# vertgenlab/gonomics

Measured on AMD Instinct MI355X. Metric: DP cells/sec + aligned pairs/sec, affine-gap 150bp x 10kb batch, higher is better.
Workload: dtype int32

## Files before the change

gonomics_amd/_lib.py:

```python
import ctypes
import os

import numpy as np

_HERE = os.path.dirname(os.path.abspath(__file__))
LIB_PATH = os.environ.get("GNX_LIB_PATH") or os.path.join(_HERE, "libgonomics_align_hip.so")

GNX_OK, GNX_EINVAL, GNX_EBASE, GNX_EEMPTY, GNX_ERANGE, GNX_EDEVICE, GNX_ENOMEM, GNX_ECAPACITY, GNX_ETRACE, GNX_EDIVZERO, GNX_ESTALE = range(11)
GNX_AFFINE_GAP, GNX_CONST_GAP, GNX_AFFINE_GAP_HIGHMEM, GNX_AFFINE_GAP_LOCAL, GNX_CONST_GAP_HIGHMEM = range(5)

EXPORTS = ["gnx_device_count", "gnx_init", "gnx_shutdown", "gnx_last_error", "gnx_free", "gnx_align_batch",
           "gnx_align_batch_windows", "gnx_align_pair", "gnx_align_batch_device", "gnx_get_timing",
           "gnx_affine_gap_chunk_batch", "gnx_multiple_affine_gap_batch", "gnx_gsw_extend_batch",
           "gnx_init_devices", "gnx_n_devices", "gnx_set_reference", "gnx_set_reference_synthetic", "gnx_align_batch_by_offset",
           "gnx_seed_index_build", "gnx_seed_index_set", "gnx_seed_find_batch", "gnx_seed_index_set_gen", "gnx_seed_find_batch_gen", "gnx_gsw_graph_create", "gnx_gsw_graph_free", "gnx_gsw_map_reads", "gnx_debug_occupy", "gnx_debug_counter", "gnx_debug_fill_scratch", "gnx_debug_gapless_certificate", "gnx_debug_gapless_certificate_n", "gnx_reference_info",
           "gnx_score_batch", "gnx_score_batch_windows", "gnx_score_batch_by_offset", "gnx_score_batch_device",
           "gnx_locate_batch", "gnx_locate_batch_windows", "gnx_locate_batch_by_offset",
           "gnx_locate_span_batch", "gnx_locate_span_batch_windows", "gnx_locate_span_batch_by_offset",
           "gnx_affine_gap_chunk_score_batch", "gnx_multiple_affine_gap_score_batch",
           "gnx_best_of_by_offset", "gnx_best_of_windows", "gnx_best_pair_by_offset", "gnx_best_pair_windows",
           "gnx_reference_index_build", "gnx_reference_index_info", "gnx_reference_index_get", "gnx_seed_candidates",
           "gnx_summarize_batch", "gnx_summarize_batch_windows", "gnx_summarize_batch_by_offset",
           "gnx_md_batch", "gnx_md_batch_windows", "gnx_md_batch_by_offset", "gnx_mapq_batch",
           "gnx_pileup_open", "gnx_pileup_info", "gnx_pileup_add_by_offset", "gnx_pileup_get", "gnx_pileup_calls", "gnx_pileup_close",
           "gnx_pileup_track_alleles", "gnx_pileup_allele_info", "gnx_pileup_alleles", "gnx_pileup_indel_calls",
           "gnx_pileup_alleles_norm", "gnx_pileup_indel_calls_norm",
           "gnx_pileup_track_qualities", "gnx_pileup_qual_info", "gnx_pileup_add_by_offset_qual", "gnx_pileup_get_qual", "gnx_pileup_genotypes"]
GNX_XCOL_EQ, GNX_XCOL_X = 3, 4


class GnxCigar(ctypes.Structure):
    _fields_ = [("run_length", ctypes.c_int64), ("op", ctypes.c_uint8), ("_pad", ctypes.c_uint8 * 7)]


CIGAR_DTYPE = np.dtype({"names": ["run_length", "op"], "formats": [np.int64, np.uint8], "offsets": [0, 8], "itemsize": 16})


class GnxParams(ctypes.Structure):
    _fields_ = [("mode", ctypes.c_int32), ("_reserved", ctypes.c_int32), ("scores", ctypes.c_int64 * 25),
                ("gap_open", ctypes.c_int64), ("gap_extend", ctypes.c_int64),
                ("checkersize_i", ctypes.c_int64), ("checkersize_j", ctypes.c_int64)]


class GnxTiming(ctypes.Structure):
    _fields_ = [("fill_ms", ctypes.c_double), ("traceback_ms", ctypes.c_double), ("total_ms", ctypes.c_double),
                ("cells", ctypes.c_int64), ("n_launches", ctypes.c_int64), ("trace_bytes", ctypes.c_int64),
                ("dominant_ms", ctypes.c_double), ("dominant_launches", ctypes.c_int64), ("fast_path", ctypes.c_int32),
                ("_pad", ctypes.c_int32), ("host_ms", ctypes.c_double), ("stage0_ms", ctypes.c_double), ("fetch_ms", ctypes.c_double),
# ... 202 lines not shown
            L.gnx_pileup_genotypes.argtypes = [ctypes.POINTER(GnxGenoOpts), ctypes.POINTER(c_p), ctypes.POINTER(i64)]
            L.gnx_pileup_genotypes.restype = ctypes.c_int
        L.gnx_seed_index_build.argtypes = [c_p, c_p, i64, ctypes.c_int, ctypes.c_int, ctypes.POINTER(c_p), ctypes.POINTER(c_p), ctypes.POINTER(i64)]
        L.gnx_seed_index_build.restype = ctypes.c_int
        L.gnx_seed_index_set.argtypes = [c_p, c_p, i64, c_p, c_p, i64, ctypes.c_int]
        L.gnx_seed_index_set.restype = ctypes.c_int
        L.gnx_seed_find_batch.argtypes = [c_p, c_p, i64, ctypes.POINTER(c_p), ctypes.POINTER(c_p)]
        L.gnx_seed_find_batch.restype = ctypes.c_int
        L.gnx_seed_index_set_gen.argtypes = [c_p, c_p, i64, c_p, c_p, i64, ctypes.c_int, ctypes.POINTER(ctypes.c_uint64)]
        L.gnx_seed_index_set_gen.restype = ctypes.c_int
        L.gnx_seed_find_batch_gen.argtypes = [ctypes.c_uint64, c_p, c_p, i64, ctypes.POINTER(c_p), ctypes.POINTER(c_p)]
        L.gnx_seed_find_batch_gen.restype = ctypes.c_int
        if hasattr(L, "gnx_gsw_map_reads"):
            L.gnx_gsw_graph_create.argtypes = [c_p, c_p, i64, c_p, c_p, i64, ctypes.c_int, ctypes.c_int, ctypes.POINTER(c_p)]
            L.gnx_gsw_graph_create.restype = ctypes.c_int
            L.gnx_gsw_graph_free.argtypes = [c_p]
            L.gnx_gsw_graph_free.restype = None
            L.gnx_gsw_map_reads.argtypes = [c_p, c_p, c_p, i64, ctypes.c_int, c_p, i64, ctypes.c_int, ctypes.POINTER(c_p), ctypes.POINTER(c_p), ctypes.POINTER(c_p)]
            L.gnx_gsw_map_reads.restype = ctypes.c_int
        L.gnx_get_timing.argtypes = [ctypes.POINTER(GnxTiming)]
        L.gnx_get_timing.restype = ctypes.c_int
        if hasattr(L, "gnx_debug_occupy"):
            L.gnx_debug_occupy.argtypes = [ctypes.c_int, ctypes.c_int]
            L.gnx_debug_occupy.restype = ctypes.c_int
        if hasattr(L, "gnx_debug_counter"):
            L.gnx_debug_counter.argtypes = [ctypes.c_int, ctypes.c_int, ctypes.POINTER(ctypes.c_int64)]
            L.gnx_debug_counter.restype = ctypes.c_int
        if hasattr(L, "gnx_debug_gapless_certificate"):
            L.gnx_debug_gapless_certificate.argtypes = [ctypes.POINTER(GnxParams), c_p, i64, c_p, i64, i64, c_p]
            L.gnx_debug_gapless_certificate.restype = ctypes.c_int
        if hasattr(L, "gnx_debug_gapless_certificate_n"):
            L.gnx_debug_gapless_certificate_n.argtypes = [ctypes.POINTER(GnxParams), c_p, i64, c_p, i64, i64, c_p]
            L.gnx_debug_gapless_certificate_n.restype = ctypes.c_int
        if hasattr(L, "gnx_debug_fill_scratch"):
            L.gnx_debug_fill_scratch.argtypes = [ctypes.c_uint32, ctypes.POINTER(ctypes.c_int64), ctypes.POINTER(ctypes.c_int64)]
            L.gnx_debug_fill_scratch.restype = ctypes.c_int
        _lib = L
    return _lib


def debug_counter(which=0, reset=True):
    v = ctypes.c_int64()
    check(lib().gnx_debug_counter(which, 1 if reset else 0, ctypes.byref(v)))
    return int(v.value)


def debug_fill_scratch(pattern):
    nb, by = ctypes.c_int64(), ctypes.c_int64()
    check(lib().gnx_debug_fill_scratch(ctypes.c_uint32(int(pattern) & 0xFFFFFFFF), ctypes.byref(nb), ctypes.byref(by)))
    return int(nb.value), int(by.value)


def debug_gapless_certificate(params, a, b, K=16):
    a = np.ascontiguousarray(a, dtype=np.uint8)
    b = np.ascontiguousarray(b, dtype=np.uint8)
    out = np.zeros(4, dtype=np.int64)
    check(lib().gnx_debug_gapless_certificate(ctypes.byref(params), a.ctypes.data, a.shape[0], b.ctypes.data, b.shape[0], int(K), out.ctypes.data))
    return bool(out[0]), int(out[1]), int(out[2]), int(out[3])


def debug_gapless_certificate_n(params, a, b, K=16):
    a = np.ascontiguousarray(a, dtype=np.uint8)
    b = np.ascontiguousarray(b, dtype=np.uint8)
    out = np.zeros(6, dtype=np.int64)
    check(lib().gnx_debug_gapless_certificate_n(ctypes.byref(params), a.ctypes.data, a.shape[0], b.ctypes.data, b.shape[0], int(K), out.ctypes.data))
    return bool(out[0]), int(out[1]), int(out[2]), int(out[3]), bool(out[4]), int(out[5])


def check(rc):
    if rc != GNX_OK:
        raise GnxError(rc, lib().gnx_last_error().decode("utf-8", "replace"))


def make_params(mode, scores, gap_open, gap_extend=0, checkersize_i=10000, checkersize_j=10000):
    p = GnxParams()
    p.mode = mode
    flat = [int(v) for row in scores for v in row]
    if len(flat) != 25:
        raise ValueError("scores must be a 5x5 matrix")
    for k, v in enumerate(flat):
        p.scores[k] = v
    p.gap_open = int(gap_open)
    p.gap_extend = int(gap_extend)
    p.checkersize_i = int(checkersize_i)
    p.checkersize_j = int(checkersize_j)
    return p


def _u8(a):
    return np.ascontiguousarray(a, dtype=np.uint8)


def _i64(a):
    return np.ascontiguousarray(a, dtype=np.int64)


def _take(ops_p, off_p, n_pairs):
    L = lib()
    off = np.ctypeslib.as_array(ctypes.cast(off_p, ctypes.POINTER(ctypes.c_int64)), shape=(n_pairs + 1,)).copy()
# ... 847 lines not shown
```

gonomics_amd/csrc/fp_cert.hip.h:

```cpp
#pragma once
#include "gnx_common.hip.h"
#include "fp_cert_decide.h"

namespace {
constexpr int CERT_K = 16;
constexpr int CERT_SLOTS = 512;
constexpr int CERT_NMAX = 160;
constexpr int CERT_CHUNK = (CERT_NMAX + 63) / 64;

__device__ __forceinline__ int64_t cert_wave_sum(int64_t v) {
#pragma unroll
    for (int d = 32; d >= 1; d >>= 1) v += __shfl_xor(v, d, 64);
    return v;
}
__device__ __forceinline__ int64_t cert_wave_scan(int64_t v, int lane) {
#pragma unroll
    for (int d = 1; d < 64; d <<= 1) { const int64_t t = __shfl_up(v, d, 64); if (lane >= d) v += t; }
    return v;
}

__device__ __forceinline__ unsigned cert_hash(unsigned code) { return code * 0x9E3779B1u; }
__device__ __forceinline__ unsigned cert_pack4(unsigned w) {
    unsigned x = w & 0x03030303u;
    x = (x | (x >> 6)) & 0x000F000Fu;
    return (x | (x >> 12)) & 0xFFu;
}

template <bool PK>
__global__ __launch_bounds__(64) void fp_cert_kernel(const PairPlan *__restrict__ plans, int n_pairs,
                                                     const uint8_t *__restrict__ a_buf, const int64_t *__restrict__ a_start,
                                                     const uint8_t *__restrict__ b_buf, const int64_t *__restrict__ b_start,
                                                     KParams kp, TbParams tp, GnxCertMatrix mx, gnx_cigar *__restrict__ stage, int cap,
                                                     int64_t *__restrict__ score_out, int64_t *__restrict__ nops,
                                                     int64_t *__restrict__ live, int64_t *__restrict__ n_cert, int *__restrict__ err) {
    __shared__ unsigned keys[CERT_SLOTS];
    __shared__ int qv[CERT_SLOTS];
    __shared__ unsigned filt[CERT_SLOTS];
    __shared__ uint8_t sa[CERT_NMAX];
    __shared__ int64_t sw[40];
    const int p = (int)blockIdx.x;
    if (p >= n_pairs) return;
    const int lane = threadIdx.x;
    const PairPlan pl = plans[p];
    const int n = pl.n, m = pl.m;
    bool bad = false;
    bool out = n < CERT_K || n > CERT_NMAX || m < n + 2 || kp.o4 >= 0 || tp.ci < n || tp.cj < m;
    BetaSrcT<PK ? 1 : 0> bp;
    const int64_t boff = b_start[pl.src];
    bp.init(b_buf, kp, boff, m);
    if (PK && bp.dirty) out = true;
    if (out) { if (lane == 0) live[p] = 1; return; }
// ... 84 lines not shown
    int64_t loss[CERT_CHUNK];
#pragma unroll
    for (int k = 0; k < CERT_CHUNK; k++) {
        const int i = i0 + k;
        loss[k] = 0;
        if (k < chunk && i < n) loss[k] = gnx_certn_lane_row<8>(&ln, sw, mx.R[4], 1, i, sa[i], (unsigned)bp.at(c + i), (unsigned)bp.at(i), (unsigned)bp.at(m - n + i));
    }
    if (__any(!ln.ok)) { if (lane == 0) live[p] = 1; return; }
    int nu = 0;
#pragma unroll
    for (int k = 0; k < CERT_CHUNK; k++) nu += __popcll(__ballot(ln.nn > k));
    const int64_t D = cert_wave_sum(ln.loss), mid_sum = cert_wave_sum(ln.mid);
    const int64_t Fi = cert_wave_scan(ln.f, lane), Gi = cert_wave_scan(ln.g, lane);
    const int f_pos = __any(ln.rows > 0 && Fi - ln.f + ln.f_top > 0);
    int64_t g_low = ln.rows > 0 ? Gi - ln.g + ln.g_low : INT64_MAX;
    int g_row = ln.rows > 0 ? ln.g_row : n;
#pragma unroll
    for (int d = 32; d >= 1; d >>= 1) gnx_cert_low_min(&g_low, &g_row, __shfl_xor(g_low, d, 64), __shfl_xor(g_row, d, 64));
    const GnxCertBounds t = gnx_certn_bounds(mx.lambda, mx.o, n, CERT_K, D, nu);
    int64_t h1 = 0, h2 = 0, t1 = 0, t2 = 0;
    if (t.edge) {
#pragma unroll
        for (int k = 0; k < CERT_CHUNK; k++) {
            const int i = i0 + k;
            if (i < t.T1) h1 += loss[k];
            if (i < t.T2) h2 += loss[k];
            if (i >= n - t.T1) t1 += loss[k];
            if (i >= n - t.T2) t2 += loss[k];
        }
        h1 = cert_wave_sum(h1); h2 = cert_wave_sum(h2); t1 = cert_wave_sum(t1); t2 = cert_wave_sum(t2);
    }
    int64_t best, ds, sc;
    gnx_cert_tail(__shfl(Gi, 63, 64), g_low, g_row, n, &best, &ds);
    if (!gnx_cert_finish(&t, mx.o, mx.e, n, m, f_pos, mid_sum, h1, h2, t1, t2, best, ds, &ds, &sc)) { if (lane == 0) live[p] = 1; return; }
    if (lane == 0) {
        gnx_cigar *stg = stage + (int64_t)p * cap;
        int cnt = 0;
        auto put = [&](int op, int64_t run) { gnx_cigar g; g.run_length = run; g.op = (uint8_t)op; for (int z = 0; z < 7; z++) g._pad[z] = 0; stg[cnt++] = g; };
        if (ds > 0) put(0, ds);
        put(1, (int64_t)m - n - c);
        put(0, (int64_t)n - ds);
        put(1, c);
        nops[p] = cnt;
        score_out[p] = sc;
        live[p] = 0;
        if (nu > 0) atomicAdd(reinterpret_cast<unsigned long long *>(n_cert), 1ull);
    }
}

__global__ __launch_bounds__(256) void fp_cert_gather_kernel(int n_pairs, const int64_t *__restrict__ live, const int64_t *__restrict__ off,
                                                             const PairPlan *__restrict__ plans, int *__restrict__ list, PairPlan *__restrict__ out) {
    const int p = blockIdx.x * blockDim.x + threadIdx.x;
    if (p >= n_pairs || !live[p]) return;
    const int64_t k = off[p];
    list[k] = p;
    out[k] = plans[p];
}

}
```

gonomics_amd/csrc/fp_cert_decide.h:

```cpp
#pragma once
#include <stdint.h>

#if defined(__HIPCC__) || defined(__CUDACC__)
#define GNX_CERT_HD __host__ __device__
#else
#define GNX_CERT_HD
#endif

struct GnxCertMatrix {
    int64_t w[25];
    int64_t R[5];
    int64_t lambda;
    int64_t o, e;
    int32_t ok;
};

GNX_CERT_HD inline void gnx_cert_matrix_init(GnxCertMatrix *mx, const int64_t *scores, int64_t gap_open, int64_t gap_extend) {
    mx->o = gap_open; mx->e = gap_extend;
    for (int x = 0; x < 25; x++) mx->w[x] = scores[x] - 2 * gap_extend;
    int ok = gap_open < 0 ? 1 : 0;
    int64_t lam = INT64_MAX;
    for (int x = 0; x < 4; x++) {
        const int64_t Rx = mx->w[x * 5 + x];
        int64_t worst = INT64_MIN;
        for (int y = 0; y < 5; y++) if (y != x && mx->w[x * 5 + y] > worst) worst = mx->w[x * 5 + y];
        mx->R[x] = Rx;
        if (Rx <= 0 || Rx <= worst) ok = 0;
        const int64_t loss = Rx - worst < Rx ? Rx - worst : Rx;
        if (loss < lam) lam = loss;
    }
    int64_t rn = 0;
    for (int y = 0; y < 5; y++) if (mx->w[20 + y] > rn) rn = mx->w[20 + y];
    mx->R[4] = rn;
    mx->lambda = lam;
    mx->ok = (ok && lam > 0) ? 1 : 0;
}

GNX_CERT_HD inline int64_t gnx_cert_table8_entry(const GnxCertMatrix *mx, int k) { return (k & 7) < 5 ? mx->w[(k >> 3) * 5 + (k & 7)] : 0; }

struct GnxCertRow {
// ... 98 lines not shown
        nu += a[i] == 4 ? 1 : 0;
        deficit += r.loss;
        mid_sum += r.mid;
        F += r.f;
        if (F > 0) return 0;
    }
    const GnxCertBounds t = gnx_certn_bounds(mx->lambda, mx->o, n, K, deficit, nu);
    if (!t.ok) return 0;
    int64_t h1 = 0, h2 = 0, t1 = 0, t2 = 0;
    if (t.edge)
        for (int64_t i = 0; i < t.T2; i++) {
            const int64_t j = n - 1 - i;
            gnx_certn_row<5>(mx->w, rn, allow_n, a[i], bd[i], bf[i], bl[i], &r);
            gnx_certn_row<5>(mx->w, rn, allow_n, a[j], bd[j], bf[j], bl[j], &r2);
            h2 += r.loss; t2 += r2.loss;
            if (i < t.T1) { h1 += r.loss; t1 += r2.loss; }
        }
    int64_t G = 0, best = 0, ds = 0;
    for (int64_t d = 1; d <= n; d++) {
        const int64_t i = n - d;
        gnx_certn_row<5>(mx->w, rn, allow_n, a[i], bd[i], bf[i], bl[i], &r);
        G += r.g;
        if (G >= best) { best = G; ds = d; }
    }
    if (edge) *edge = t.edge;
    if (nu_out) *nu_out = nu;
    return gnx_cert_finish(&t, mx->o, mx->e, n, m, 0, mid_sum, h1, h2, t1, t2, best, ds, d_star, score);
}
GNX_CERT_HD inline int gnx_cert_decide(const GnxCertMatrix *mx, const uint8_t *a, int64_t n, const uint8_t *bd, const uint8_t *bf, const uint8_t *bl,
                                       int64_t m, int64_t c, int64_t K, int64_t ci, int64_t cj, int64_t *d_star, int64_t *score) {
    return gnx_certn_decide(mx, a, n, bd, bf, bl, m, c, K, ci, cj, 0, d_star, score, nullptr, nullptr);
}

inline int gnx_cert_scan_naive(const uint8_t *a, int64_t n, const uint8_t *b, int64_t m, int64_t K, int64_t *c_out) {
    int found = 0;
    int64_t c = 0;
    for (int64_t q = 0; q + K <= n; q++)
        for (int64_t j = 0; j + K <= m; j++) {
            int64_t t = 0;
            while (t < K && a[q + t] < 4 && a[q + t] == (b[j + t] & 3)) t++;
            if (t < K) continue;
            if (found && j - q != c) return 0;
            found = 1; c = j - q;
        }
    *c_out = c;
    return found;
}
```

gonomics_amd/csrc/gnx_align.hip:

```cpp
#include "gnx_common.hip.h"
#include "fill_affine.hip.h"
#include "fp_sweep.hip.h"
#include "fp_rounds.h"
#include "fill_const.hip.h"
#include "traceback.hip.h"
#include "fp_walk.hip.h"
#include "fp_cert.hip.h"
#include "aux_kernels.hip.h"
#include "const_long.hip.h"
#include "const_long_wg.hip.h"
#include "const_long_walk.hip.h"
#include "affine_long.hip.h"
#include "affine_long64.hip.h"
#include "const_long64.hip.h"
#include "farm64.hip.h"
#include "lat_fill.hip.h"
#include "lat_wide.hip.h"
#include "seed_kernels.hip.h"
#include "score_sweep.hip.h"
#include "n1_sweep.hip.h"
#include "span_origin.hip.h"
#include "ref_seeds.hip.h"
#include "aln_summary.hip.h"
#include "aln_md.hip.h"
// ... 172 lines not shown
    for (int x = 0; x < 25; x++) if (p->scores[x] > lim || p->scores[x] < -lim) { set_err("score out of int32 kernel range%s", ""); return GNX_ERANGE; }
    if (p->gap_open > lim || p->gap_open < -lim || (affine && (p->gap_extend > lim || p->gap_extend < -lim))) { set_err("gap penalty out of int32 kernel range%s", ""); return GNX_ERANGE; }
    kp.b2 = nullptr; kp.bflag = nullptr; kp.brank = nullptr; kp.bexc = nullptr;
    for (int x = 0; x < 25; x++) kp.sc4[x] = (int)(4 * p->scores[x]);
    kp.o4 = (int)(4 * p->gap_open);
    kp.e4 = affine ? (int)(4 * p->gap_extend) : 0;
    kp.oe4 = kp.o4 + kp.e4;
    kp.d00_4 = local ? 0 : kp.o4;
    kp.ecol4 = local ? 0 : kp.e4;
    kp.g4 = kp.o4;
    kp.rb_pub = RB_PUB;
    kp.ckc = CKC_SMALL;
    tp.ci = lowmem ? p->checkersize_i : ((int64_t)1 << 62);
    tp.cj = lowmem ? p->checkersize_j : ((int64_t)1 << 62);
    tp.d00 = local ? 0 : p->gap_open;
    tp.ecol = local ? 0 : p->gap_extend;
    tp.gap_open = p->gap_open;
    tp.gap_extend = affine ? p->gap_extend : 0;
    tp.affine = affine ? 1 : 0;
    return GNX_OK;
}

int64_t max_abs_pen(const gnx_params *p, bool affine) {
    int64_t mx = 0;
    for (int x = 0; x < 25; x++) mx = std::max<int64_t>(mx, llabs((long long)p->scores[x]));
    if (affine) mx = std::max<int64_t>(mx, llabs((long long)(p->gap_open + p->gap_extend)));
    mx = std::max<int64_t>(mx, llabs((long long)p->gap_open));
    if (affine) mx = std::max<int64_t>(mx, llabs((long long)p->gap_extend));
    return mx;
}

std::atomic<int64_t> g_cert_ok{0}, g_cert_offered{0};
std::atomic<int64_t> g_cert_n{0};
std::atomic<int64_t> g_fpc_hit{0}, g_fpc_miss{0};

int run_device(const gnx_params *prm, int64_t n_pairs, const uint8_t *d_a, const int64_t *d_as, const uint8_t *d_b, const int64_t *d_bs,
               const int64_t *h_alen, const int64_t *h_blen, int64_t *d_score, gnx_cigar *d_ops, int64_t ops_capacity, int64_t *d_ops_off,
               int64_t *out_total, hipStream_t stream, const int *d_smat, const int64_t *h_soff, int gsw, int2 *d_endpos, bool no_fast_path, bool smat16);

__global__ __launch_bounds__(64) void occupy_kernel(long long ticks) {
    extern __shared__ int occupy_lds[];
    occupy_lds[threadIdx.x] = (int)ticks;
    const long long t0 = wall_clock64();
    while (wall_clock64() - t0 < ticks) __builtin_amdgcn_s_sleep(64);
}

int claim_test_switch(int *sw, hipStream_t st) {
    const char *e = getenv("GNX_TICKET_DELAY"), *g = getenv("GNX_CLAIM_GRACE_US");
    if (!e || !*e) return GNX_OK;
    const int v = (std::min(std::max(atoi(e), 0), 0xffff)) | ((g && *g) ? (std::min(std::max(atoi(g), 1), 0x7fff) << 16) : 0);
    HIPCHK(hipMemcpyAsync(sw, &v, 4, hipMemcpyHostToDevice, st));
    HIPCHK(hipStreamSynchronize(st));
    return GNX_OK;
}

int launch_scan(const int64_t *d_nops, int n, int64_t *d_off, int64_t *d_carry, hipStream_t stream) {
    Ctx &c = g_ctx;
    if (n <= 8192) { hipLaunchKernelGGL(scan_kernel, dim3(1), dim3(1024), 0, stream, d_nops, n, d_off, d_carry); return GNX_OK; }
    const int nb = (n + 1023) / 1024;
    int rc;
    if ((rc = c.scan_tmp.ensure((size_t)(2 * nb + 2) * 8))) return rc;
    int64_t *sums = reinterpret_cast<int64_t *>(c.scan_tmp.p), *boff = sums + nb;
    hipLaunchKernelGGL(scan_sums_kernel, dim3((unsigned)nb), dim3(1024), 0, stream, d_nops, n, sums);
    hipLaunchKernelGGL(scan_kernel, dim3(1), dim3(1024), 0, stream, sums, nb, boff, d_carry);
    hipLaunchKernelGGL(scan_apply_kernel, dim3((unsigned)nb), dim3(1024), 0, stream, d_nops, n, boff, d_off);
    return GNX_OK;
// ... 74 lines not shown
    if (!cached || c.fpc_ptr != c.plans.p) {
        if (cached) { set_err("internal: plan cache lost its buffer%s", ""); return GNX_EINVAL; }
        HIPCHK(hipMemcpyAsync(c.plans.p, plans.data(), (size_t)np * sizeof(PairPlan), hipMemcpyHostToDevice, stream));
        HIPCHK(hipStreamSynchronize(stream));
        c.fpc_alen.assign(h_alen, h_alen + n_pairs); c.fpc_blen.assign(h_blen, h_blen + n_pairs);
        c.fpc_roff = roff; c.fpc_coff = coff; c.fpc_cells = cells; c.fpc_mmax = m_maxb; c.fpc_ptr = c.plans.p; c.fpc_rboff = rboff; c.fpc_strips = S;
    }
    (cached ? g_fpc_hit : g_fpc_miss)++;
    const PairPlan *dpl = reinterpret_cast<const PairPlan *>(c.plans.p);
    int *d_hfwd = reinterpret_cast<int *>(c.hcol.p);
    int *d_whcol = d_hfwd + np;
    unsigned *d_rowi = reinterpret_cast<unsigned *>(c.fp_rowi.p);
    unsigned *d_tail = reinterpret_cast<unsigned *>(c.fp_tail.p);
    int2 *d_ckpt = reinterpret_cast<int2 *>(c.fp_ckpt.p);
    FpState *d_st = reinterpret_cast<FpState *>(c.fp_states.p);
    gnx_cigar *d_stage = reinterpret_cast<gnx_cigar *>(c.fp_stage.p);
    int64_t *d_nops = reinterpret_cast<int64_t *>(c.nops.p);
    PairPlan *d_wpl[2] = {reinterpret_cast<PairPlan *>(c.fp_wplans[0].p), reinterpret_cast<PairPlan *>(c.fp_wplans[1].p)};
    int *d_act[2] = {reinterpret_cast<int *>(c.fp_active[0].p), reinterpret_cast<int *>(c.fp_active[1].p)};
    const dim3 blockF(64), blockT(64);
    const int max_it = getenv("GNX_FP_MAXIT") ? atoi(getenv("GNX_FP_MAXIT")) : -1;
    const int tiles_per = (int)((m_maxb + FP_TILE - 1) / FP_TILE);
    double refill_ms = 0;

    const char *certenv = getenv("GNX_FP_CERT");
    const bool cert = S == 1 && !xp && prm->gap_open < 0 && !(certenv && certenv[0] == '0') &&
                      ((certenv && certenv[0] == '2') || n_pairs > (int64_t)G8 * 3 * 4 * c.n_cu);
    int n_live = np;
    int64_t *d_cflag = nullptr, *d_coff = nullptr;
    int *d_live = nullptr;
    PairPlan *d_gpl = nullptr;
    bool gathered = false;
    if (cert) {
        if ((rc = c.fp_cflag.ensure((size_t)(2 * np + 3) * 8))) return rc;
        if ((rc = c.fp_live.ensure((size_t)np * 4))) return rc;
        if ((rc = c.fp_gplans.ensure((size_t)np * sizeof(PairPlan)))) return rc;
        d_cflag = reinterpret_cast<int64_t *>(c.fp_cflag.p); d_coff = d_cflag + np + 2;
        d_live = reinterpret_cast<int *>(c.fp_live.p);
        d_gpl = reinterpret_cast<PairPlan *>(c.fp_gplans.p);
    }
    auto certify = [&](hipStream_t st) -> int {
        GnxCertMatrix mx;
        int64_t sc64[25];
        for (int x = 0; x < 25; x++) sc64[x] = (int64_t)(kp.sc4[x] >> 2);
        gnx_cert_matrix_init(&mx, sc64, (int64_t)(kp.o4 >> 2), (int64_t)(kp.e4 >> 2));
        g_cert_offered += np;
        if (!mx.ok) return GNX_OK;
        HIPCHK(hipMemsetAsync(d_cflag + np, 0, 16, st));
        auto kc = kp.b2 ? fp_cert_kernel<true> : fp_cert_kernel<false>;
        hipLaunchKernelGGL(kc, dim3((unsigned)np), dim3(64), 0, st, dpl, np, d_a, d_as, d_b, d_bs, kp, tp, mx, d_stage, CAP, d_score, d_nops, d_cflag, d_cflag + np + 1, d_err);
        HIPCHK(hipGetLastError());
        if ((rc = launch_scan(d_cflag, np, d_coff, d_cflag + np, st))) return rc;
        hipLaunchKernelGGL(fp_cert_gather_kernel, dim3((unsigned)((np + 255) / 256)), dim3(256), 0, st, np, d_cflag, d_coff, dpl, d_live, d_gpl);
        HIPCHK(hipGetLastError());
        int64_t nl[2] = {0, 0};
        HIPCHK(hipMemcpyAsync(nl, d_cflag + np, 16, hipMemcpyDeviceToHost, st));
        HIPCHK(hipStreamSynchronize(st));
        n_live = (int)nl[0];
        gathered = true;
        g_cert_ok += np - n_live - nl[1];
        g_cert_n += nl[1];
        if (getenv("GNX_DEBUG")) fprintf(stderr, "[gnx fp] gapless certificate: %d of %d pairs certified (%d of them hold an N), %d go through the sweep\n", np - n_live, np, (int)nl[1], n_live);
        return GNX_OK;
    };

    auto forward = [&](const PairPlan *splans, int cnt, hipStream_t st) -> int {
        if (cnt <= 0) return GNX_OK;
        const dim3 grid8((unsigned)((cnt + G8 - 1) / G8));
        if (two) {
            int2 *rb = reinterpret_cast<int2 *>(c.rowbuf.p);
            const int top_rows = (int)(top_hi + G8 - 1) / G8;
            const bool pk = kp.b2 != nullptr;
            auto klev = xp ? (top_rows <= 8 ? fp_sweep_levels_kernel<8, true> : (top_rows <= 12 ? fp_sweep_levels_kernel<12, true> : (top_rows <= 16 ? fp_sweep_levels_kernel<16, true> : fp_sweep_levels_kernel<20, true>)))
                      : pk ? (top_rows <= 8 ? fp_sweep_levels_kernel<8, false, true> : (top_rows <= 12 ? fp_sweep_levels_kernel<12, false, true> : (top_rows <= 16 ? fp_sweep_levels_kernel<16, false, true> : fp_sweep_levels_kernel<20, false, true>)))
                           : (top_rows <= 8 ? fp_sweep_levels_kernel<8> : (top_rows <= 12 ? fp_sweep_levels_kernel<12> : (top_rows <= 16 ? fp_sweep_levels_kernel<16> : fp_sweep_levels_kernel<20>)));
            const int W = (int)grid8.x;
            int *prog = reinterpret_cast<int *>(c.fp_prog.p);
            if (!no_pipe()) {
                HIPCHK(hipMemsetAsync(prog, 0, ((size_t)S * W * 2 + 2) * 4, st));
                if ((rc = claim_test_switch(prog + (size_t)S * W * 2, st))) return rc;
                hipLaunchKernelGGL(klev, dim3((unsigned)(S * W)), blockF, 0, st, splans, cnt, d_a, d_as, d_b, d_bs, kp, d_hfwd, d_ckpt, d_rowi, d_tail, d_err, rb, S, W, 0, 1, prog);
                HIPCHK(hipGetLastError());
                int e = 0;
                HIPCHK(hipMemcpyAsync(&e, d_err, 4, hipMemcpyDeviceToHost, st));
                HIPCHK(hipStreamSynchronize(st));
                if (!(e & 16)) return GNX_OK;
                e &= ~16;
                HIPCHK(hipMemcpyAsync(d_err, &e, 4, hipMemcpyHostToDevice, st));
                HIPCHK(hipStreamSynchronize(st));
                if (getenv("GNX_DEBUG")) fprintf(stderr, "[gnx fp] a row block timed out waiting for the one above it -> one launch per level\n");
            }
            for (int level = 0; level < S; level++)
                hipLaunchKernelGGL(klev, grid8, blockF, 0, st, splans, cnt, d_a, d_as, d_b, d_bs, kp, d_hfwd, d_ckpt, d_rowi, d_tail, d_err, rb, S, W, level, 0, prog);
            HIPCHK(hipGetLastError());
            return GNX_OK;
// ... 3357 lines not shown
    if (rc) return rc;
    if (!a || !b || !out || n < 1 || m < 1 || K < 1 || !affine || local) { set_err("bad argument%s", ""); return GNX_EINVAL; }
    out[0] = out[1] = out[2] = out[3] = 0;
    GnxCertMatrix mx;
    gnx_cert_matrix_init(&mx, p->scores, p->gap_open, p->gap_extend);
    int64_t c = 0, ds = 0, sc = 0;
    for (int64_t j = 0; j < m; j++) if (b[j] >= 5) return GNX_OK;
    if (m < n + 2 || K > n || !gnx_cert_scan_naive(a, n, b, m, K, &c)) return GNX_OK;
    if (c <= 0 || c >= m - n) return GNX_OK;
    if (!gnx_cert_decide(&mx, a, n, b + c, b, b + (m - n), m, c, K, tp.ci, tp.cj, &ds, &sc)) return GNX_OK;
    out[0] = 1; out[1] = c; out[2] = ds; out[3] = sc;
    return GNX_OK;
}

int gnx_debug_gapless_certificate_n(const gnx_params *p, const uint8_t *a, int64_t n, const uint8_t *b, int64_t m, int64_t K, int64_t *out) {
    g_err[0] = 0;
    if (!getenv("GNX_DEBUG_ENTRY")) { set_err("gnx_debug_gapless_certificate_n is a test hook: set GNX_DEBUG_ENTRY=1%s", ""); return GNX_EINVAL; }
    KParams kp; TbParams tp; bool affine, local, lowmem;
    int rc = check_params(p, kp, tp, affine, local, lowmem);
    if (rc) return rc;
    if (!a || !b || !out || n < 1 || m < 1 || K < 1 || !affine || local) { set_err("bad argument%s", ""); return GNX_EINVAL; }
    for (int x = 0; x < 6; x++) out[x] = 0;
    GnxCertMatrix mx;
    gnx_cert_matrix_init(&mx, p->scores, p->gap_open, p->gap_extend);
    int64_t c = 0, ds = 0, sc = 0, edge = 0, nu = 0;
    for (int64_t j = 0; j < m; j++) if (b[j] >= 5) return GNX_OK;
    if (m < n + 2 || K > n || !gnx_cert_scan_naive(a, n, b, m, K, &c)) return GNX_OK;
    if (c <= 0 || c >= m - n) return GNX_OK;
    if (!gnx_certn_decide(&mx, a, n, b + c, b, b + (m - n), m, c, K, tp.ci, tp.cj, 1, &ds, &sc, &edge, &nu)) return GNX_OK;
    out[0] = 1; out[1] = c; out[2] = ds; out[3] = sc; out[4] = edge; out[5] = nu;
    return GNX_OK;
}

int gnx_debug_counter(int which, int reset, int64_t *out) {
    ApiCall api;
    CtxScope sc(ctx_at(0));
    if (which < 0 || which > 13 || !out) { set_err("bad argument%s", ""); return GNX_EINVAL; }
    if (which >= 12) {
        std::atomic<int64_t> &v = which == 12 ? g_fpc_hit : g_fpc_miss;
        *out = v.load();
        if (reset) v = 0;
        return GNX_OK;
    }
    if (which >= 9) {
        std::atomic<int64_t> &v = which == 9 ? g_cert_ok : (which == 10 ? g_cert_offered : g_cert_n);
        *out = v.load();
        if (reset) v = 0;
        return GNX_OK;
    }
    if (which >= 7) {
        std::atomic<int64_t> &v = which == 7 ? g_sv_lds : g_sv_slab;
        *out = v.load();
        if (reset) v = 0;
        return GNX_OK;
    }
    if (which == 1 || which == 2) {
        *out = which == 1 ? g_pq_batches.load() : g_pq_pairs.load();
        if (reset) { if (which == 1) g_pq_batches = 0; else g_pq_pairs = 0; }
        return GNX_OK;
    }
    if (which >= 5) { *out = which == 5 ? g_last_w64_r.load() : g_last_w64_ck.load(); return GNX_OK; }
    int rc = ensure_init();
    if (rc) return rc;
    HIPCHK(hipSetDevice(g_ctx.device));
    HIPCHK(hipDeviceSynchronize());
    unsigned long long v = 0;
    if (which >= 3) {
        unsigned long long q[2] = {0, 0};
        HIPCHK(hipMemcpyFromSymbol(q, HIP_SYMBOL(g_dev_q1), sizeof(q)));
        if (reset) { const unsigned long long z[2] = {0, 0}; HIPCHK(hipMemcpyToSymbol(HIP_SYMBOL(g_dev_q1), z, sizeof(z))); }
// ... 20 lines not shown
```

include/gnx_align.h:

```cpp
#ifndef GNX_ALIGN_H
#define GNX_ALIGN_H

#include <stdint.h>

#ifdef __cplusplus
extern "C" {
#endif

#define GNX_OK 0
#define GNX_EINVAL 1
#define GNX_EBASE 2
#define GNX_EEMPTY 3
#define GNX_ERANGE 4
#define GNX_EDEVICE 5
#define GNX_ENOMEM 6
#define GNX_ECAPACITY 7
#define GNX_ETRACE 8
#define GNX_EDIVZERO 9
#define GNX_ESTALE 10

#define GNX_COL_M 0
#define GNX_COL_I 1
#define GNX_COL_D 2

// ... 224 lines not shown
    int32_t  depth;
    uint8_t  ref, _pad2[3];
} gnx_pile_indel_call;
int gnx_pileup_track_alleles(int64_t reserve_events);
int gnx_pileup_allele_info(int32_t *out_tracking, int64_t *out_events, int64_t *out_device_bytes);
int gnx_pileup_alleles(gnx_pile_allele **out, int64_t *out_n);
int gnx_pileup_indel_calls(const gnx_pile_call_opts *o, gnx_pile_indel_call **out_calls, int64_t *out_n);
int gnx_pileup_alleles_norm(gnx_pile_allele **out, int64_t *out_n);
int gnx_pileup_indel_calls_norm(const gnx_pile_call_opts *o, gnx_pile_indel_call **out_calls, int64_t *out_n);

typedef struct gnx_geno_opts { int32_t min_depth, min_qual, prior_het, prior_hom, _reserved[2]; } gnx_geno_opts;
typedef struct gnx_pile_genotype {
    int64_t pos;
    int32_t pl[3];
    int32_t gq, qual;
    int32_t depth, ref_count, alt_count, alt_fwd;
    uint8_t gt, ref, alt, _pad;
} gnx_pile_genotype;
int gnx_pileup_track_qualities(int32_t min_baseq);
int gnx_pileup_qual_info(int32_t *out_tracking, int32_t *out_min_baseq, int64_t *out_device_bytes);
int gnx_pileup_add_by_offset_qual(const gnx_params *p, int64_t n_pairs, const uint8_t *read_cat, const int64_t *read_off,
                                  const int64_t *ref_start, const int64_t *ref_len, const uint8_t *strand,
                                  const gnx_cigar *ops, const int64_t *ops_off, const uint8_t *use ,
                                  const uint8_t *qual_cat);
int gnx_pileup_get_qual(int64_t first, int64_t count, int32_t *out );
int gnx_pileup_genotypes(const gnx_geno_opts *o, gnx_pile_genotype **out, int64_t *out_n);

int gnx_get_timing(gnx_timing *out);
int gnx_debug_occupy(int n_workgroups, int milliseconds);
int gnx_debug_counter(int which, int reset, int64_t *out);
int gnx_debug_fill_scratch(uint32_t pattern, int64_t *out_buffers, int64_t *out_bytes);
int gnx_debug_gapless_certificate(const gnx_params *p, const uint8_t *a, int64_t n, const uint8_t *b, int64_t m, int64_t K, int64_t *out);
int gnx_debug_gapless_certificate_n(const gnx_params *p, const uint8_t *a, int64_t n, const uint8_t *b, int64_t m, int64_t K, int64_t *out);

int gnx_affine_gap_chunk_batch(const gnx_params *p, int64_t chunk_size, int64_t n_pairs,
                               const uint8_t *alpha_cat, const int64_t *alpha_off, const uint8_t *beta_cat, const int64_t *beta_off,
                               int64_t *out_score, gnx_cigar **out_ops, int64_t **out_ops_off);

int gnx_multiple_affine_gap_batch(const gnx_params *p, int64_t chunk_size, int64_t n_groups, const uint8_t *group_bases,
                                  const int64_t *group_off, const int32_t *group_nseq, const int64_t *group_len,
                                  int64_t n_pairs, const int32_t *pair_a, const int32_t *pair_b,
                                  int64_t *out_score, gnx_cigar **out_ops, int64_t **out_ops_off);

int gnx_affine_gap_chunk_score_batch(const gnx_params *p, int64_t chunk_size, int64_t n_pairs,
                                     const uint8_t *alpha_cat, const int64_t *alpha_off, const uint8_t *beta_cat, const int64_t *beta_off,
                                     int64_t *out_score);
int gnx_multiple_affine_gap_score_batch(const gnx_params *p, int64_t chunk_size, int64_t n_groups, const uint8_t *group_bases,
                                        const int64_t *group_off, const int32_t *group_nseq, const int64_t *group_len,
                                        int64_t n_pairs, const int32_t *pair_a, const int32_t *pair_b, int64_t *out_score);

#define GNX_GSW_LEFT 0
#define GNX_GSW_RIGHT 1
int gnx_gsw_extend_batch(int side, const int64_t *scores, int64_t gap_pen, int64_t n_pairs,
                         const uint8_t *alpha_cat, const int64_t *alpha_off, const uint8_t *beta_cat, const int64_t *beta_off,
                         int64_t *out_score, int64_t *out_end_i, int64_t *out_end_j, gnx_cigar **out_ops, int64_t **out_ops_off);

typedef struct gnx_gsw_graph gnx_gsw_graph;
typedef struct gnx_giraf {
    int64_t q_start, q_end, t_start, t_end, aln_score;
    int64_t node_off, n_nodes;
    int64_t cigar_off, n_cigar;
    int32_t pos_strand, flag, map_q, has_cigar;
    int32_t seq_is_rc;
    int32_t panicked;
} gnx_giraf;
int gnx_gsw_graph_create(const uint8_t *node_cat, const int64_t *node_off, int64_t n_nodes, const int32_t *edge_from, const int32_t *edge_to,
// ... 26 lines not shown
```

Before: 10600 billion.

## Add graded edge rule to gapless certificate so more pairs skip DP sweep

After: 12180 billion (median of 6 runs). +15.0%, better.

```diff
diff --git a/gonomics_amd/_lib.py b/gonomics_amd/_lib.py
--- a/gonomics_amd/_lib.py
+++ b/gonomics_amd/_lib.py
@@ -13,7 +13,7 @@
            "gnx_align_batch_windows", "gnx_align_pair", "gnx_align_batch_device", "gnx_get_timing",
            "gnx_affine_gap_chunk_batch", "gnx_multiple_affine_gap_batch", "gnx_gsw_extend_batch",
            "gnx_init_devices", "gnx_n_devices", "gnx_set_reference", "gnx_set_reference_synthetic", "gnx_align_batch_by_offset",
-           "gnx_seed_index_build", "gnx_seed_index_set", "gnx_seed_find_batch", "gnx_seed_index_set_gen", "gnx_seed_find_batch_gen", "gnx_gsw_graph_create", "gnx_gsw_graph_free", "gnx_gsw_map_reads", "gnx_debug_occupy", "gnx_debug_counter", "gnx_debug_fill_scratch", "gnx_debug_gapless_certificate", "gnx_debug_gapless_certificate_n", "gnx_reference_info",
+           "gnx_seed_index_build", "gnx_seed_index_set", "gnx_seed_find_batch", "gnx_seed_index_set_gen", "gnx_seed_find_batch_gen", "gnx_gsw_graph_create", "gnx_gsw_graph_free", "gnx_gsw_map_reads", "gnx_debug_occupy", "gnx_debug_counter", "gnx_debug_fill_scratch", "gnx_debug_gapless_certificate", "gnx_debug_gapless_certificate_n", "gnx_debug_gapless_certificate_edge", "gnx_reference_info",
            "gnx_score_batch", "gnx_score_batch_windows", "gnx_score_batch_by_offset", "gnx_score_batch_device",
            "gnx_locate_batch", "gnx_locate_batch_windows", "gnx_locate_batch_by_offset",
            "gnx_locate_span_batch", "gnx_locate_span_batch_windows", "gnx_locate_span_batch_by_offset",
@@ -282,6 +282,9 @@
         if hasattr(L, "gnx_debug_gapless_certificate_n"):
             L.gnx_debug_gapless_certificate_n.argtypes = [ctypes.POINTER(GnxParams), c_p, i64, c_p, i64, i64, c_p]
             L.gnx_debug_gapless_certificate_n.restype = ctypes.c_int
+        if hasattr(L, "gnx_debug_gapless_certificate_edge"):
+            L.gnx_debug_gapless_certificate_edge.argtypes = [ctypes.POINTER(GnxParams), c_p, i64, c_p, i64, i64, c_p]
+            L.gnx_debug_gapless_certificate_edge.restype = ctypes.c_int
         if hasattr(L, "gnx_debug_fill_scratch"):
             L.gnx_debug_fill_scratch.argtypes = [ctypes.c_uint32, ctypes.POINTER(ctypes.c_int64), ctypes.POINTER(ctypes.c_int64)]
             L.gnx_debug_fill_scratch.restype = ctypes.c_int
@@ -315,6 +318,14 @@
     out = np.zeros(6, dtype=np.int64)
     check(lib().gnx_debug_gapless_certificate_n(ctypes.byref(params), a.ctypes.data, a.shape[0], b.ctypes.data, b.shape[0], int(K), out.ctypes.data))
     return bool(out[0]), int(out[1]), int(out[2]), int(out[3]), bool(out[4]), int(out[5])
+
+
+def debug_gapless_certificate_edge(params, a, b, K=16):
+    a = np.ascontiguousarray(a, dtype=np.uint8)
+    b = np.ascontiguousarray(b, dtype=np.uint8)
+    out = np.zeros(8, dtype=np.int64)
+    check(lib().gnx_debug_gapless_certificate_edge(ctypes.byref(params), a.ctypes.data, a.shape[0], b.ctypes.data, b.shape[0], int(K), out.ctypes.data))
+    return bool(out[0]), int(out[1]), int(out[2]), int(out[3]), bool(out[4]), int(out[5]), bool(out[6]), int(out[7])
 
 
 def check(rc):
diff --git a/gonomics_amd/csrc/fp_cert.hip.h b/gonomics_amd/csrc/fp_cert.hip.h
--- a/gonomics_amd/csrc/fp_cert.hip.h
+++ b/gonomics_amd/csrc/fp_cert.hip.h
@@ -17,6 +17,17 @@
 #pragma unroll
     for (int d = 1; d < 64; d <<= 1) { const int64_t t = __shfl_up(v, d, 64); if (lane >= d) v += t; }
     return v;
+}
+
+__device__ __forceinline__ int cert_wave_scan32(int v, int lane) {
+#pragma unroll
+    for (int d = 1; d < 64; d <<= 1) { const int t = __shfl_up(v, d, 64); if (lane >= d) v += t; }
+    return v;
+}
+__device__ __forceinline__ int64_t cert_read_lane64(int64_t v, int src) {
+    const int s = __builtin_amdgcn_readfirstlane(src);
+    const unsigned lo = (unsigned)__builtin_amdgcn_readlane((int)(unsigned)(uint64_t)v, s), hi = (unsigned)__builtin_amdgcn_readlane((int)(unsigned)((uint64_t)v >> 32), s);
+    return (int64_t)(((uint64_t)hi << 32) | lo);
 }
 
 __device__ __forceinline__ unsigned cert_hash(unsigned code) { return code * 0x9E3779B1u; }
@@ -167,7 +178,44 @@
     }
     int64_t best, ds, sc;
     gnx_cert_tail(__shfl(Gi, 63, 64), g_low, g_row, n, &best, &ds);
-    if (!gnx_cert_finish(&t, mx.o, mx.e, n, m, f_pos, mid_sum, h1, h2, t1, t2, best, ds, &ds, &sc)) { if (lane == 0) live[p] = 1; return; }
+    bool by_edge = false;
+    if (!gnx_cert_finish(&t, mx.o, mx.e, n, m, f_pos, mid_sum, h1, h2, t1, t2, best, ds, &ds, &sc)) {
+        if (!(t.ok && !f_pos && t.edge && ds < n && (h1 + t2 >= -mx.o || h2 + t1 >= -mx.o))) { if (lane == 0) live[p] = 1; return; }
+        GnxCertEdgeLane el;
+        gnx_certe_lane_init(&el, i0);
+#pragma unroll
+        for (int k = 0; k < CERT_CHUNK; k++) {
+            const int i = i0 + k;
+            if (k < chunk && i < n) gnx_certe_lane_row(&el, sa[i], (unsigned)bp.at(i), (unsigned)bp.at(m - n + i));
+        }
+        const int inc0 = cert_wave_scan32(el.c0, lane), incm = cert_wave_scan32(el.cm, lane);
+        const int before0 = inc0 - el.c0, afterm = __builtin_amdgcn_readlane(incm, 63) - incm;
+        const int64_t k0 = cert_wave_scan(ln.loss, lane) - ln.loss;
+        auto prefix = [&](int k) -> int64_t {
+            if (k >= n) return D;
+            const int L = k / chunk, r = k - L * chunk;
+            int64_t v = k0;
+#pragma unroll
+            for (int x = 0; x + 1 < CERT_CHUNK; x++) v += r > x ? loss[x] : 0;
+            return cert_read_lane64(v, L);
+        };
+        const int J30 = (int)gnx_certe_grades(mx.lambda, mx.o, D);
+        bool pass = true;
+        for (int j = 0; j <= J30 && pass; j++) {
+            const int hr = gnx_certe_head_row(&el, before0, j), tr = gnx_certe_tail_row(&el, afterm, j);
+            const unsigned long long bh = __ballot(hr >= 0), bt = __ballot(tr >= 0);
+            const int A0 = bh ? __builtin_amdgcn_readlane(hr, __builtin_amdgcn_readfirstlane(__ffsll(bh) - 1)) : n;
+            const int Am = bt ? n - 1 - __builtin_amdgcn_readlane(tr, __builtin_amdgcn_readfirstlane(__ffsll(bt) - 1)) : n;
+            int64_t pq[4], ha, ta, hb, tb;
+            gnx_certe_corners(CERT_K, nu, j, A0, Am, pq);
+            gnx_certe_span(n, pq[0], pq[1], &ha, &ta);
+            gnx_certe_span(n, pq[2], pq[3], &hb, &tb);
+            pass = gnx_certe_grade(mx.lambda, mx.o, j, prefix((int)ha) + D - prefix((int)ta), prefix((int)hb) + D - prefix((int)tb)) != 0;
+        }
+        if (!pass) { if (lane == 0) live[p] = 1; return; }
+        sc = mid_sum + best + 2 * mx.o + mx.e * ((int64_t)n + m);
+        by_edge = true;
+    }
     if (lane == 0) {
         gnx_cigar *stg = stage + (int64_t)p * cap;
         int cnt = 0;
@@ -179,7 +227,8 @@
         nops[p] = cnt;
         score_out[p] = sc;
         live[p] = 0;
-        if (nu > 0) atomicAdd(reinterpret_cast<unsigned long long *>(n_cert), 1ull);
+        if (by_edge) atomicAdd(reinterpret_cast<unsigned long long *>(n_cert + 1), 1ull);
+        else if (nu > 0) atomicAdd(reinterpret_cast<unsigned long long *>(n_cert), 1ull);
     }
 }
 
diff --git a/gonomics_amd/csrc/fp_cert_decide.h b/gonomics_amd/csrc/fp_cert_decide.h
--- a/gonomics_amd/csrc/fp_cert_decide.h
+++ b/gonomics_amd/csrc/fp_cert_decide.h
@@ -6,6 +6,7 @@
 #else
 #define GNX_CERT_HD
 #endif
+#define GNX_CERTE_HD GNX_CERT_HD __attribute__((always_inline))
 
 struct GnxCertMatrix {
     int64_t w[25];
@@ -170,6 +171,103 @@
     return gnx_certn_decide(mx, a, n, bd, bf, bl, m, c, K, ci, cj, 0, d_star, score, nullptr, nullptr);
 }
 
+GNX_CERTE_HD inline void gnx_certe_flags(unsigned a, unsigned bf, unsigned bl, int *nf0, int *nfm) {
+    *nf0 = (a != 4 && a != bf) ? 1 : 0;
+    *nfm = (a != 4 && a != bl) ? 1 : 0;
+}
+struct GnxCertEdgeLane {
+    int32_t bits0, bitsm, c0, cm, i0, rows;
+};
+GNX_CERTE_HD inline void gnx_certe_lane_init(GnxCertEdgeLane *l, int i0) { l->bits0 = l->bitsm = l->c0 = l->cm = 0; l->i0 = i0; l->rows = 0; }
+GNX_CERTE_HD inline void gnx_certe_lane_row(GnxCertEdgeLane *l, unsigned a, unsigned bf, unsigned bl) {
+    int f0, fm;
+    gnx_certe_flags(a, bf, bl, &f0, &fm);
+    l->bits0 |= f0 << l->rows; l->bitsm |= fm << l->rows;
+    l->c0 += f0; l->cm += fm;
+    l->rows++;
+}
+GNX_CERTE_HD inline int gnx_certe_head_row(const GnxCertEdgeLane *l, int before0, int j) {
+    int r = j - before0;
+    if (r < 0 || r >= l->c0) return -1;
+    for (int k = 0; k < l->rows; k++) if ((l->bits0 >> k) & 1) { if (r == 0) return l->i0 + k; r--; }
+    return -1;
+}
+GNX_CERTE_HD inline int gnx_certe_tail_row(const GnxCertEdgeLane *l, int afterm, int j) {
+    int r = j - afterm;
+    if (r < 0 || r >= l->cm) return -1;
+    for (int k = l->rows - 1; k >= 0; k--) if ((l->bitsm >> k) & 1) { if (r == 0) return l->i0 + k; r--; }
+    return -1;
+}
+GNX_CERTE_HD inline void gnx_certe_corners(int64_t K, int64_t nu, int64_t j, int64_t A0, int64_t Am, int64_t pq[4]) {
+    const int64_t Ts = (1 + j + nu) * (K - 1) + j + nu, Tt = (2 + j + nu) * (K - 1) + j + nu;
+    pq[0] = A0 < Ts ? A0 : Ts; pq[1] = Ts + Am < Tt ? Ts + Am : Tt;
+    pq[2] = Ts + A0 < Tt ? Ts + A0 : Tt; pq[3] = Am < Ts ? Am : Ts;
+}
+GNX_CERTE_HD inline void gnx_certe_span(int64_t n, int64_t p, int64_t q, int64_t *head, int64_t *tail) {
+    const int64_t pp = p < n ? p : n, qq = q < n - pp ? q : n - pp;
+    *head = pp; *tail = n - qq;
+}
+GNX_CERTE_HD inline int gnx_certe_grade(int64_t lambda, int64_t o, int64_t j, int64_t e1, int64_t e2) {
+    const int64_t lim = -o + lambda * j;
+    return (e1 < lim && e2 < lim) ? 1 : 0;
+}
+GNX_CERTE_HD inline int64_t gnx_certe_grades(int64_t lambda, int64_t o, int64_t D) { return gnx_cert_div(D + o, lambda); }
+
+GNX_CERT_HD inline int gnx_certe_decide(const GnxCertMatrix *mx, const uint8_t *a, int64_t n, const uint8_t *bd, const uint8_t *bf, const uint8_t *bl,
+                                        int64_t m, int64_t c, int64_t K, int64_t ci, int64_t cj, int allow_n, int64_t *d_star, int64_t *score,
+                                        int64_t *edge, int64_t *nu_out, int64_t *by_edge, int64_t *jdec) {
+    if (by_edge) *by_edge = 0;
+    if (jdec) *jdec = -1;
+    if (gnx_certn_decide(mx, a, n, bd, bf, bl, m, c, K, ci, cj, allow_n, d_star, score, edge, nu_out)) return 1;
+    if (!mx->ok || n < 1 || K < 1 || m < n + 2 || c <= 0 || c >= m - n || ci < n || cj < m) return 0;
+    const int64_t rn = mx->R[4];
+    GnxCertRow r;
+    int64_t D = 0, mid_sum = 0, F = 0, nu = 0;
+    for (int64_t i = 0; i < n; i++) {
+        if (!gnx_certn_row<5>(mx->w, rn, allow_n, a[i], bd[i], bf[i], bl[i], &r)) return 0;
+        nu += a[i] == 4 ? 1 : 0;
+        D += r.loss; mid_sum += r.mid; F += r.f;
+        if (F > 0) return 0;
+    }
+    const GnxCertBounds t = gnx_certn_bounds(mx->lambda, mx->o, n, K, D, nu);
+    if (!t.ok || !t.edge) return 0;
+    int64_t G = 0, best = 0, ds = 0;
+    for (int64_t d = 1; d <= n; d++) {
+        gnx_certn_row<5>(mx->w, rn, allow_n, a[n - d], bd[n - d], bf[n - d], bl[n - d], &r);
+        G += r.g;
+        if (G >= best) { best = G; ds = d; }
+    }
+    if (ds >= n) return 0;
+    auto E = [&](int64_t p, int64_t q) -> int64_t {
+        int64_t head, tail, s = 0;
+        gnx_certe_span(n, p, q, &head, &tail);
+        for (int64_t i = 0; i < n; i++)
+            if (i < head || i >= tail) { gnx_certn_row<5>(mx->w, rn, allow_n, a[i], bd[i], bf[i], bl[i], &r); s += r.loss; }
+        return s;
+    };
+    const int64_t J30 = gnx_certe_grades(mx->lambda, mx->o, D);
+    for (int64_t j = 0; j <= J30; j++) {
+        int64_t A0 = n, Am = n, seen = 0;
+        int f0, fm;
+        for (int64_t i = 0; i < n; i++) { gnx_certe_flags(a[i], bf[i], bl[i], &f0, &fm); if (f0 && seen++ == j) { A0 = i; break; } }
+        seen = 0;
+        for (int64_t i = n - 1; i >= 0; i--) { gnx_certe_flags(a[i], bf[i], bl[i], &f0, &fm); if (fm && seen++ == j) { Am = n - 1 - i; break; } }
+        int64_t pq[4];
+        gnx_certe_corners(K, nu, j, A0, Am, pq);
+        if (!gnx_certe_grade(mx->lambda, mx->o, j, E(pq[0], pq[1]), E(pq[2], pq[3]))) return 0;
+        if (jdec) {
+            gnx_certe_corners(K, nu, j, n, n, pq);
+            if (!gnx_certe_grade(mx->lambda, mx->o, j, E(pq[0], pq[1]), E(pq[2], pq[3]))) *jdec = j;
+        }
+    }
+    *d_star = ds;
+    *score = mid_sum + best + 2 * mx->o + mx->e * (n + m);
+    if (edge) *edge = 1;
+    if (nu_out) *nu_out = nu;
+    if (by_edge) *by_edge = 1;
+    return 1;
+}
+
 inline int gnx_cert_scan_naive(const uint8_t *a, int64_t n, const uint8_t *b, int64_t m, int64_t K, int64_t *c_out) {
     int found = 0;
     int64_t c = 0;
diff --git a/gonomics_amd/csrc/gnx_align.hip b/gonomics_amd/csrc/gnx_align.hip
--- a/gonomics_amd/csrc/gnx_align.hip
+++ b/gonomics_amd/csrc/gnx_align.hip
@@ -228,6 +228,7 @@
 
 std::atomic<int64_t> g_cert_ok{0}, g_cert_offered{0};
 std::atomic<int64_t> g_cert_n{0};
+std::atomic<int64_t> g_cert_edge{0};
 std::atomic<int64_t> g_fpc_hit{0}, g_fpc_miss{0};
 
 int run_device(const gnx_params *prm, int64_t n_pairs, const uint8_t *d_a, const int64_t *d_as, const uint8_t *d_b, const int64_t *d_bs,
@@ -368,10 +369,10 @@
     PairPlan *d_gpl = nullptr;
     bool gathered = false;
     if (cert) {
-        if ((rc = c.fp_cflag.ensure((size_t)(2 * np + 3) * 8))) return rc;
+        if ((rc = c.fp_cflag.ensure((size_t)(2 * np + 4) * 8))) return rc;
         if ((rc = c.fp_live.ensure((size_t)np * 4))) return rc;
         if ((rc = c.fp_gplans.ensure((size_t)np * sizeof(PairPlan)))) return rc;
-        d_cflag = reinterpret_cast<int64_t *>(c.fp_cflag.p); d_coff = d_cflag + np + 2;
+        d_cflag = reinterpret_cast<int64_t *>(c.fp_cflag.p); d_coff = d_cflag + np + 3;
         d_live = reinterpret_cast<int *>(c.fp_live.p);
         d_gpl = reinterpret_cast<PairPlan *>(c.fp_gplans.p);
     }
@@ -382,21 +383,22 @@
         gnx_cert_matrix_init(&mx, sc64, (int64_t)(kp.o4 >> 2), (int64_t)(kp.e4 >> 2));
         g_cert_offered += np;
         if (!mx.ok) return GNX_OK;
-        HIPCHK(hipMemsetAsync(d_cflag + np, 0, 16, st));
+        HIPCHK(hipMemsetAsync(d_cflag + np, 0, 24, st));
         auto kc = kp.b2 ? fp_cert_kernel<true> : fp_cert_kernel<false>;
         hipLaunchKernelGGL(kc, dim3((unsigned)np), dim3(64), 0, st, dpl, np, d_a, d_as, d_b, d_bs, kp, tp, mx, d_stage, CAP, d_score, d_nops, d_cflag, d_cflag + np + 1, d_err);
         HIPCHK(hipGetLastError());
         if ((rc = launch_scan(d_cflag, np, d_coff, d_cflag + np, st))) return rc;
         hipLaunchKernelGGL(fp_cert_gather_kernel, dim3((unsigned)((np + 255) / 256)), dim3(256), 0, st, np, d_cflag, d_coff, dpl, d_live, d_gpl);
         HIPCHK(hipGetLastError());
-        int64_t nl[2] = {0, 0};
-        HIPCHK(hipMemcpyAsync(nl, d_cflag + np, 16, hipMemcpyDeviceToHost, st));
+        int64_t nl[3] = {0, 0, 0};
+        HIPCHK(hipMemcpyAsync(nl, d_cflag + np, 24, hipMemcpyDeviceToHost, st));
         HIPCHK(hipStreamSynchronize(st));
         n_live = (int)nl[0];
         gathered = true;
-        g_cert_ok += np - n_live - nl[1];
+        g_cert_ok += np - n_live - nl[1] - nl[2];
         g_cert_n += nl[1];
-        if (getenv("GNX_DEBUG")) fprintf(stderr, "[gnx fp] gapless certificate: %d of %d pairs certified (%d of them hold an N), %d go through the sweep\n", np - n_live, np, (int)nl[1], n_live);
+        g_cert_edge += nl[2];
+        if (getenv("GNX_DEBUG")) fprintf(stderr, "[gnx fp] gapless certificate: %d of %d pairs certified (%d of them hold an N, %d by the graded edge rule only), %d go through the sweep\n", np - n_live, np, (int)nl[1], (int)nl[2], n_live);
         return GNX_OK;
     };
 
@@ -3820,10 +3822,35 @@
     return GNX_OK;
 }
 
+int gnx_debug_gapless_certificate_edge(const gnx_params *p, const uint8_t *a, int64_t n, const uint8_t *b, int64_t m, int64_t K, int64_t *out) {
+    g_err[0] = 0;
+    if (!getenv("GNX_DEBUG_ENTRY")) { set_err("gnx_debug_gapless_certificate_edge is a test hook: set GNX_DEBUG_ENTRY=1%s", ""); return GNX_EINVAL; }
+    KParams kp; TbParams tp; bool affine, local, lowmem;
+    int rc = check_params(p, kp, tp, affine, local, lowmem);
+    if (rc) return rc;
+    if (!a || !b || !out || n < 1 || m < 1 || K < 1 || !affine || local) { set_err("bad argument%s", ""); return GNX_EINVAL; }
+    for (int x = 0; x < 8; x++) out[x] = 0;
+    out[7] = -1;
+    GnxCertMatrix mx;
+    gnx_cert_matrix_init(&mx, p->scores, p->gap_open, p->gap_extend);
+    int64_t c = 0, ds = 0, sc = 0, edge = 0, nu = 0, by_edge = 0, jdec = -1;
+    for (int64_t j = 0; j < m; j++) if (b[j] >= 5) return GNX_OK;
+    if (m < n + 2 || K > n || !gnx_cert_scan_naive(a, n, b, m, K, &c)) return GNX_OK;
+    if (c <= 0 || c >= m - n) return GNX_OK;
+    if (!gnx_certe_decide(&mx, a, n, b + c, b, b + (m - n), m, c, K, tp.ci, tp.cj, 1, &ds, &sc, &edge, &nu, &by_edge, &jdec)) return GNX_OK;
+    out[0] = 1; out[1] = c; out[2] = ds; out[3] = sc; out[4] = edge; out[5] = nu; out[6] = by_edge; out[7] = jdec;
+    return GNX_OK;
+}
+
 int gnx_debug_counter(int which, int reset, int64_t *out) {
     ApiCall api;
     CtxScope sc(ctx_at(0));
-    if (which < 0 || which > 13 || !out) { set_err("bad argument%s", ""); return GNX_EINVAL; }
+    if (which < 0 || which > 14 || !out) { set_err("bad argument%s", ""); return GNX_EINVAL; }
+    if (which == 14) {
+        *out = g_cert_edge.load();
+        if (reset) g_cert_edge = 0;
+        return GNX_OK;
+    }
     if (which >= 12) {
         std::atomic<int64_t> &v = which == 12 ? g_fpc_hit : g_fpc_miss;
         *out = v.load();
diff --git a/include/gnx_align.h b/include/gnx_align.h
--- a/include/gnx_align.h
+++ b/include/gnx_align.h
@@ -280,6 +280,7 @@
 int gnx_debug_fill_scratch(uint32_t pattern, int64_t *out_buffers, int64_t *out_bytes);
 int gnx_debug_gapless_certificate(const gnx_params *p, const uint8_t *a, int64_t n, const uint8_t *b, int64_t m, int64_t K, int64_t *out);
 int gnx_debug_gapless_certificate_n(const gnx_params *p, const uint8_t *a, int64_t n, const uint8_t *b, int64_t m, int64_t K, int64_t *out);
+int gnx_debug_gapless_certificate_edge(const gnx_params *p, const uint8_t *a, int64_t n, const uint8_t *b, int64_t m, int64_t K, int64_t *out);
 
 int gnx_affine_gap_chunk_batch(const gnx_params *p, int64_t chunk_size, int64_t n_pairs,
                                const uint8_t *alpha_cat, const int64_t *alpha_off, const uint8_t *beta_cat, const int64_t *beta_off,
```
